# YiZhiXiaoGuLI/xerus

Measured on AMD Instinct MI355X. Metric: GFLOP/s on TT contraction + TT-round sweep time, order-10 rank-256, higher is better.
Workload: dtype f64; 1 GPU; TT order-10 n=20 rank-256: <x,y> + x.round(256) per step; order=10, mode_size=20, rank=256, parallelism=replicas x1

## Files before the change

include/xerus_amd.h:

```cpp
#ifndef XERUS_AMD_H
#define XERUS_AMD_H

#include <stddef.h>
#include <stdint.h>

#ifdef __cplusplus
extern "C" {
#endif

typedef struct xrs_handle_s* xrs_handle_t;

#define XRS_OK 0
#define XRS_EINVAL (-1)
#define XRS_ENOMEM (-2)
#define XRS_EHIP (-3)
#define XRS_ENUMERIC 1

int xrs_create(xrs_handle_t* handle, int device);
int xrs_destroy(xrs_handle_t handle);
int xrs_set_stream(xrs_handle_t handle, void* hip_stream);
void* xrs_get_stream(xrs_handle_t handle);
int xrs_synchronize(xrs_handle_t handle);
const char* xrs_last_error(void);
const char* xrs_version(void);
// ... 8 lines not shown

int xrs_nrm2(xrs_handle_t handle, double* result, const double* x, size_t n);
int xrs_dot(xrs_handle_t handle, double* result, const double* x, const double* y, size_t n);
int xrs_asum(xrs_handle_t handle, double* result, const double* x, size_t n);
int xrs_scal(xrs_handle_t handle, double* x, double alpha, size_t n);
int xrs_axpy(xrs_handle_t handle, double* y, double alpha, const double* x, size_t n);
int xrs_scale_rows(xrs_handle_t handle, double* X, const double* s, size_t m, size_t n);

int xrs_gemm(xrs_handle_t handle, double* C, size_t M, size_t N, double alpha,
             const double* A, size_t lda, int transA, size_t K,
             const double* B, size_t ldb, int transB);

int xrs_gemm_batched(xrs_handle_t handle, size_t count, double* const* C, size_t M, size_t N, double alpha,
                     const double* const* A, size_t lda, int transA, size_t K,
                     const double* const* B, size_t ldb, int transB);

int xrs_gemm_sym(xrs_handle_t handle, double* C, size_t N, double alpha,
                 const double* A, size_t lda, int transA, size_t K,
                 const double* B, size_t ldb, int transB);

int xrs_gemm_forms(xrs_handle_t handle, size_t count, double* const* C, size_t M, size_t N, double alpha,
                   const double* const* A, size_t lda, int transA, size_t K,
                   const double* const* B, size_t ldb, int transB, int sym, int tri);

int xrs_gemm_f32(xrs_handle_t handle, float* C, size_t M, size_t N, float alpha,
                 const float* A, size_t lda, int transA, size_t K,
                 const float* B, size_t ldb, int transB);

int xrs_permute(xrs_handle_t handle, double* out, const double* in, size_t ndim,
                const size_t* dims, const size_t* shuffle);

int xrs_qc(xrs_handle_t handle, double* Q, double* C, size_t* rank, const double* A, size_t m, size_t n);
int xrs_cq(xrs_handle_t handle, double* C, double* Q, size_t* rank, const double* A, size_t m, size_t n);
int xrs_qr(xrs_handle_t handle, double* Q, double* R, const double* A, size_t m, size_t n);
int xrs_rq(xrs_handle_t handle, double* R, double* Q, const double* A, size_t m, size_t n);
int xrs_svd(xrs_handle_t handle, double* U, double* S, double* Vt, const double* A, size_t m, size_t n);
int xrs_svd_batched(xrs_handle_t handle, double* U, double* S, double* Vt, int* status,
                    const double* A, size_t batch, size_t m, size_t n);
int xrs_svd_batched_fits(size_t m, size_t n);
int xrs_solve(xrs_handle_t handle, double* X, const double* A, size_t m, size_t n, const double* B, size_t p);
int xrs_solve_least_squares(xrs_handle_t handle, double* X, const double* A, size_t m, size_t n, const double* B, size_t p);
int xrs_svd_rows_vt(xrs_handle_t handle, double* S, double* Vt, int* sweeps, const double* A, size_t p, size_t q, int kernel);
int xrs_sym_tridiag(xrs_handle_t handle, double* d, double* e, const double* A, size_t n);
int xrs_sym_eig_top(xrs_handle_t handle, double* lam, double* Ut, int* status, const double* A, size_t n, size_t kk);


// ... 111 lines not shown
```

xerus_amd/capi.py:

```python
from __future__ import annotations

import ctypes as C
import os
from typing import Sequence

import numpy as np

_HERE = os.path.dirname(os.path.abspath(__file__))
LIB_PATH = os.environ.get("XRS_LIB_PATH") or os.path.join(_HERE, "libxerus_amd.so")

_SZ = C.c_size_t
_DP = C.c_void_p

SIGNATURES = {
    "xrs_create": (C.c_int, [C.POINTER(_DP), C.c_int]),
    "xrs_destroy": (C.c_int, [_DP]),
    "xrs_set_stream": (C.c_int, [_DP, _DP]),
    "xrs_get_stream": (_DP, [_DP]),
    "xrs_synchronize": (C.c_int, [_DP]),
    "xrs_last_error": (C.c_char_p, []),
    "xrs_version": (C.c_char_p, []),
    "xrs_malloc": (C.c_int, [_DP, C.POINTER(_DP), _SZ]),
    "xrs_free": (C.c_int, [_DP, _DP]),
    "xrs_pool_bytes": (_SZ, [_DP]),
    "xrs_upload": (C.c_int, [_DP, _DP, _DP, _SZ]),
    "xrs_download": (C.c_int, [_DP, _DP, _DP, _SZ]),
    "xrs_memset_zero": (C.c_int, [_DP, _DP, _SZ]),
    "xrs_copy": (C.c_int, [_DP, _DP, _DP, _SZ]),
    "xrs_nrm2": (C.c_int, [_DP, C.POINTER(C.c_double), _DP, _SZ]),
    "xrs_dot": (C.c_int, [_DP, C.POINTER(C.c_double), _DP, _DP, _SZ]),
    "xrs_asum": (C.c_int, [_DP, C.POINTER(C.c_double), _DP, _SZ]),
    "xrs_scal": (C.c_int, [_DP, _DP, C.c_double, _SZ]),
    "xrs_axpy": (C.c_int, [_DP, _DP, C.c_double, _DP, _SZ]),
    "xrs_scale_rows": (C.c_int, [_DP, _DP, _DP, _SZ, _SZ]),
    "xrs_gemm": (C.c_int, [_DP, _DP, _SZ, _SZ, C.c_double, _DP, _SZ, C.c_int, _SZ, _DP, _SZ, C.c_int]),
    "xrs_gemm_f32": (C.c_int, [_DP, _DP, _SZ, _SZ, C.c_float, _DP, _SZ, C.c_int, _SZ, _DP, _SZ, C.c_int]),
    "xrs_gemm_sym": (C.c_int,[_DP, _DP, _SZ, C.c_double, _DP, _SZ, C.c_int, _SZ, _DP, _SZ, C.c_int]),
    "xrs_gemm_batched": (C.c_int, [_DP, _SZ, C.POINTER(_DP), _SZ, _SZ, C.c_double, C.POINTER(_DP), _SZ, C.c_int, _SZ,
                                   C.POINTER(_DP), _SZ, C.c_int]),
    "xrs_gemm_forms": (C.c_int, [_DP, _SZ, C.POINTER(_DP), _SZ, _SZ, C.c_double, C.POINTER(_DP), _SZ, C.c_int, _SZ,
                                 C.POINTER(_DP), _SZ, C.c_int, C.c_int, C.c_int]),
    "xrs_permute": (C.c_int, [_DP, _DP, _DP, _SZ, C.POINTER(_SZ), C.POINTER(_SZ)]),
    "xrs_qc": (C.c_int, [_DP, _DP, _DP, C.POINTER(_SZ), _DP, _SZ, _SZ]),
    "xrs_cq": (C.c_int, [_DP, _DP, _DP, C.POINTER(_SZ), _DP, _SZ, _SZ]),
    "xrs_qr": (C.c_int, [_DP, _DP, _DP, _DP, _SZ, _SZ]),
    "xrs_rq": (C.c_int, [_DP, _DP, _DP, _DP, _SZ, _SZ]),
    "xrs_svd": (C.c_int, [_DP, _DP, _DP, _DP, _DP, _SZ, _SZ]),
    "xrs_svd_batched": (C.c_int, [_DP, _DP, _DP, _DP, C.POINTER(C.c_int), _DP, _SZ, _SZ, _SZ]),
    "xrs_svd_batched_fits": (C.c_int, [_SZ, _SZ]),
    "xrs_solve": (C.c_int, [_DP, _DP, _DP, _SZ, _SZ, _DP, _SZ]),
    "xrs_solve_least_squares": (C.c_int, [_DP, _DP, _DP, _SZ, _SZ, _DP, _SZ]),
    "xrs_svd_rows_vt": (C.c_int, [_DP, _DP, _DP, C.POINTER(C.c_int), _DP, _SZ, _SZ, C.c_int]),
    "xrs_sym_eig_top": (C.c_int, [_DP, _DP, _DP, C.POINTER(C.c_int), _DP, _SZ, _SZ]),
    "xrs_sym_tridiag": (C.c_int, [_DP, _DP, _DP, _DP, _SZ]),
    "xrs_tt_entrywise_product": (C.c_int, [_DP, _SZ, C.POINTER(_SZ), C.POINTER(_SZ), C.POINTER(_DP), C.POINTER(_SZ), C.POINTER(_DP),
                                           C.c_double, C.POINTER(_DP)]),
    "xrs_tt_entrywise_square": (C.c_int, [_DP, _SZ, C.POINTER(_SZ), C.POINTER(_SZ), C.POINTER(_DP), C.c_double, C.POINTER(_DP),
                                          C.POINTER(_SZ)]),
    "xrs_tt_rank_one_argmax": (C.c_int, [_DP, _SZ, C.POINTER(_SZ), C.POINTER(_DP), C.POINTER(_SZ)]),
    "xrs_tt_operator_apply": (C.c_int, [_DP, _SZ, C.POINTER(_SZ), C.POINTER(_SZ), C.POINTER(_SZ), C.POINTER(_SZ), C.POINTER(_DP),
                                        C.POINTER(_SZ), C.POINTER(_DP), C.c_int, C.POINTER(_DP)]),
    "xrs_tt_move_core": (C.c_int, [_DP, _SZ, C.POINTER(_SZ), C.POINTER(_SZ), C.POINTER(_DP), C.c_int, _SZ, _SZ, C.c_int]),
    "xrs_tt_round": (C.c_int, [_DP, _SZ, C.POINTER(_SZ), C.POINTER(_SZ), C.POINTER(_DP), C.c_int, _SZ,
                               C.POINTER(_SZ), C.c_double]),
# ... 159 lines not shown
    def gemm_f32(self, C_: "Float32Array", M, N, alpha, A: "Float32Array", lda, transA, K, B: "Float32Array", ldb, transB):
        _check("xrs_gemm_f32", self.lib.xrs_gemm_f32(self.h, _DP(C_.ptr), M, N, float(alpha), _DP(A.ptr), lda, int(transA),
                                                    K, _DP(B.ptr), ldb, int(transB)))

    def array_f32(self, a: np.ndarray) -> "Float32Array":
        return Float32Array.from_host(self, a)

    def gemm_sym(self, C_: "DeviceArray", N, alpha, A: "DeviceArray", lda, transA, K, B: "DeviceArray", ldb, transB):
        _check("xrs_gemm_sym", self.lib.xrs_gemm_sym(self.h, _DP(C_.ptr), N, alpha, _DP(A.ptr), lda, int(transA), K,
                                                    _DP(B.ptr), ldb, int(transB)))

    def gemm_batched(self, Cs, M, N, alpha, As, lda, transA, K, Bs, ldb, transB):
        cnt = len(Cs)
        tab = lambda xs: (_DP * max(1, cnt))(*[_DP(x.ptr) for x in xs])
        _check("xrs_gemm_batched", self.lib.xrs_gemm_batched(self.h, cnt, tab(Cs), M, N, alpha, tab(As), lda, int(transA),
                                                            K, tab(Bs), ldb, int(transB)))

    def gemm_forms(self, Cs, M, N, alpha, As, lda, transA, K, Bs, ldb, transB, sym: bool = False, tri: int = 0):
        cnt = len(Cs)
        tab = lambda xs: (_DP * max(1, cnt))(*[_DP(x.ptr) for x in xs])
        _check("xrs_gemm_forms", self.lib.xrs_gemm_forms(self.h, cnt, tab(Cs), M, N, alpha, tab(As), lda, int(transA), K,
                                                        tab(Bs), ldb, int(transB), int(sym), int(tri)))

    def tangent_to_tt(self, n, r, Us, Vs, add_base: bool):
        d = len(n)
        tab = lambda xs: (_DP * d)(*[_DP(x.ptr) for x in xs])
        out = (_DP * d)()
        _check("xrs_tt_tangent_to_tt", self.lib.xrs_tt_tangent_to_tt(self.h, d, _arr(n), _arr(r), tab(Us), tab(Vs),
                                                                    int(add_base), out))
        cores = []
        for k in range(d):
            shape = (2 * r[k] if k else 1, n[k], 2 * r[k + 1] if k + 1 < d else 1)
            c = DeviceArray(self, shape, ptr=out[k])
            c.owned = True
            cores.append(c)
        return cores

    def matmul(self, A: "DeviceArray", transA: bool, B: "DeviceArray", transB: bool, alpha: float = 1.0):
        am, ak = (A.shape[1], A.shape[0]) if transA else (A.shape[0], A.shape[1])
        bk, bn = (B.shape[1], B.shape[0]) if transB else (B.shape[0], B.shape[1])
        assert ak == bk, (A.shape, B.shape)
        out = self.empty((am, bn))
        self.gemm(out, am, bn, alpha, A, A.shape[1], transA, ak, B, B.shape[1], transB)
        return out

    def permute(self, out: "DeviceArray", inp: "DeviceArray", dims, shuffle):
# ... 495 lines not shown
```

xerus_amd/csrc/elementwise.hpp:

```cpp
#pragma once
#include <algorithm>

#include "runtime.hpp"

namespace xrs {

void reduce_to_device(xrs_handle_t h, int mode, const double* x, const double* y, size_t n, double* out_dev,
                      double* partial = nullptr);
double reduce_to_host(xrs_handle_t h, int mode, const double* x, const double* y, size_t n);
void scal(xrs_handle_t h, double* x, double alpha, size_t n);
void axpy(xrs_handle_t h, double* y, double alpha, const double* x, size_t n);
void ldexp_copy(xrs_handle_t h, double* dst, const double* src, int ex, size_t n);
constexpr int kAmaxMany = 64;
void amax_enqueue(xrs_handle_t h, const double* const* x, const size_t* n, int count, double* out_dev);
void norms_enqueue(xrs_handle_t h, const double* const* x, const size_t* n, int count, double* out_dev);
int range_exponent(double am);
int range_exponent(xrs_handle_t h, const double* A, size_t n);
void scale_rows(xrs_handle_t h, double* X, const double* s, size_t m, size_t n);
void scale_cols(xrs_handle_t h, double* X, const double* s, size_t m, size_t n);
void diag_sum(xrs_handle_t h, double* out, const double* X, size_t P, size_t m);
void offset_add(xrs_handle_t h, double* out, const size_t* out_dims, const double* in, const size_t* in_dims, size_t nd,
                const size_t* offsets, double alpha);
void strided_eval(xrs_handle_t h, double* out, const double* in, size_t nd, const size_t* out_dims, const size_t* in_strides,
                  size_t nt, const size_t* tr_dims, const size_t* tr_strides, size_t base);

constexpr int kTriA = 1, kTriB = 2;
void gemm(xrs_handle_t h, double* C, size_t M, size_t N, double alpha, const double* A, size_t lda, bool ta, size_t K,
          const double* B, size_t ldb, bool tb, int tri = 0);
constexpr int kGemmBatchMax = 32;
void gemm_batched(xrs_handle_t h, int count, double* const* C, size_t M, size_t N, double alpha, const double* const* A,
                  size_t lda, bool ta, size_t K, const double* const* B, size_t ldb, bool tb, bool sym = false,
                  int tri = 0);
void gemm_sym(xrs_handle_t h, double* C, size_t N, double alpha, const double* A, size_t lda, bool ta, size_t K,
              const double* B, size_t ldb, bool tb);

struct GemmSpec {
    const double* A;
    const double* B;
    double* C;
    size_t M, N, K, lda, ldb;
    bool ta, tb;
};
inline void gemm(xrs_handle_t h, const GemmSpec& g) {
    gemm(h, g.C, g.M, g.N, 1.0, g.A, g.lda, g.ta, g.K, g.B, g.ldb, g.tb);
}

void permute(xrs_handle_t h, double* out, const double* in, size_t ndim, const size_t* dims, const size_t* shuffle);

}
```

xerus_amd/csrc/gemm.hip:

```cpp
#include <algorithm>
#include <type_traits>
#include <utility>
#include <cstdio>
#include <cstdlib>

#include <hip/hip_ext.h>

#include "elementwise.hpp"
#include "runtime.hpp"

namespace xrs {

typedef double d4 __attribute__((ext_vector_type(4)));

struct GemmOne {
    const double* A;
    const double* B;
    double* C;
    __host__ __device__ const double* a(int) const { return A; }
    __host__ __device__ const double* b(int) const { return B; }
    __device__ double* c(int) const { return C; }
};
struct GemmMany {
    const double* A[kGemmBatchMax];
    const double* B[kGemmBatchMax];
    double* C[kGemmBatchMax];
    __host__ __device__ const double* a(int i) const { return A[i]; }
    __host__ __device__ const double* b(int i) const { return B[i]; }
    __device__ double* c(int i) const { return C[i]; }
};

template <int BM, int BN, int WGM, int WGN, int WGK>
constexpr int gemm_min_waves() { return (BM * BN >= 128 * 128) ? 2 : 4; }

#ifdef XRS_GEMM_TRACE
__device__ unsigned long long* g_gemm_trace = nullptr;
__device__ unsigned long long* g_gemm_steps = nullptr;
#define XRS_TRACE_BEGIN                                                   \
    const unsigned long long xrs_t0 = __builtin_amdgcn_s_memrealtime();  \
    const unsigned long long xrs_c0 = __builtin_amdgcn_s_memtime();
#define XRS_TRACE_STEP(t)                                                                                   \
    if (threadIdx.x == 0 && g_gemm_steps != nullptr && (t) < 15) {                                          \
        const size_t wg = blockIdx.x + size_t(gridDim.x) * (blockIdx.y + size_t(gridDim.y) * blockIdx.z);   \
        g_gemm_steps[16 * wg + (t)] = __builtin_amdgcn_s_memtime() - xrs_c0;                                \
    }
#define XRS_TRACE_END                                                                                     \
    if (threadIdx.x == 0 && g_gemm_trace != nullptr) {                                                    \
        const size_t wg = blockIdx.x + size_t(gridDim.x) * (blockIdx.y + size_t(gridDim.y) * blockIdx.z); \
        const unsigned long long t1 = __builtin_amdgcn_s_memrealtime();                                   \
        const unsigned hw = __builtin_amdgcn_s_getreg((31 << 11) | 4);                 \
        const unsigned xcc = __builtin_amdgcn_s_getreg((31 << 11) | 20);              \
        g_gemm_trace[3 * wg] = xrs_t0;                                                                   \
        g_gemm_trace[3 * wg + 1] = t1;                                                                   \
        g_gemm_trace[3 * wg + 2] = (static_cast<unsigned long long>(xcc) << 32) | hw;                    \
        if (g_gemm_steps != nullptr) g_gemm_steps[16 * wg + 15] = __builtin_amdgcn_s_memtime() - xrs_c0;  \
    }
#else
#define XRS_TRACE_BEGIN
#define XRS_TRACE_END
#define XRS_TRACE_STEP(t)
#endif

template <int BM, int BN, int GBK, int WGM, int WGN, int WGK, int PD, bool TA, bool TB, class PTR>
__device__ __forceinline__ void gemm_body(const PTR& ptrs, size_t lda, size_t ldb, int M, int N, int K, int kps,
                                          double alpha, double* __restrict__ slab, int tiles_m, int xcd_group,
                                          int* __restrict__ tickets, int sym);

template <int BM, int BN, int GBK, int WGM, int WGN, int WGK, int PD, bool TA, bool TB, class PTR>
__global__ void __launch_bounds__(WGM * WGN * WGK * 64, (gemm_min_waves<BM, BN, WGM, WGN, WGK>()))
k_gemm_f64(const PTR ptrs, size_t lda, size_t ldb, int M, int N, int K, int kps, double alpha,
           double* __restrict__ slab, int tiles_m, int xcd_group, int* __restrict__ tickets, int sym) {
    XRS_TRACE_BEGIN
    gemm_body<BM, BN, GBK, WGM, WGN, WGK, PD, TA, TB, PTR>(ptrs, lda, ldb, M, N, K, kps, alpha, slab, tiles_m,
                                                          xcd_group, tickets, sym);
    XRS_TRACE_END
}

template <int TM, int TN, int WGM, int WGN, int WGK, int NACC, class PTR>
__device__ __forceinline__ void gemm_finish(d4 (&acc2)[NACC][TM][TN], double* lds, const PTR& ptrs, int M, int N,
                                            double alpha, double* __restrict__ slab, int* __restrict__ tickets,
                                            int sym, int m0, int n0, int wm, int wn, int kg, int pos, int xb, int yb, int zb) {
    const int bz = yb;
    double* __restrict__ C = ptrs.c(bz);
    const int zslice = bz * int(gridDim.z) + zb;
    const int tslot = bz * int(gridDim.x) + xb;
    const int tid = threadIdx.x;
    const int lane = tid & 63;
    const bool mirror = sym != 0;
    d4 acc[TM][TN];
#pragma unroll
    for (int i = 0; i < TM; ++i)
#pragma unroll
        for (int j = 0; j < TN; ++j) {
            acc[i][j] = acc2[0][i][j];
            if constexpr (NACC > 1) acc[i][j] += acc2[1][i][j];
        }
    if constexpr (WGK > 1) {
        double* red = lds;
        if (kg > 0) {
#pragma unroll
            for (int i = 0; i < TM; ++i)
#pragma unroll
                for (int j = 0; j < TN; ++j)
#pragma unroll
                    for (int r = 0; r < 4; ++r)
                        red[((((kg - 1) * (WGM * WGN) + pos) * TM * TN + i * TN + j) * 4 + r) * 64 + lane] = acc[i][j][r];
        }
        __syncthreads();
// ... 23 lines not shown
#pragma unroll
                for (int r = 0; r < 4; ++r) {
                    const int row = m0 + wm + i * 16 + lg + 4 * r;
                    if (row < M && col < N) {
                        if (tickets != nullptr)
                            __hip_atomic_store(&out[size_t(row) * N + col], acc[i][j][r], __ATOMIC_RELAXED,
                                               __HIP_MEMORY_SCOPE_AGENT);
                        else if (!mirror || to_slab)
                            out[size_t(row) * N + col] = scale * acc[i][j][r];
                        else if (row >= col) {
                            out[size_t(row) * N + col] = scale * acc[i][j][r];
                            out[size_t(col) * N + row] = scale * acc[i][j][r];
                        }
                    }
                }
            }
    }
    if (tickets == nullptr) return;
    asm volatile("s_waitcnt vmcnt(0)" ::: "memory");
    __syncthreads();
    double* flag = lds;
    if (tid == 0) {
        const int t = __hip_atomic_fetch_add(&tickets[tslot], 1, __ATOMIC_RELAXED, __HIP_MEMORY_SCOPE_AGENT);
        const bool last = (t == int(gridDim.z) - 1);
        if (last) __hip_atomic_store(&tickets[tslot], 0, __ATOMIC_RELAXED, __HIP_MEMORY_SCOPE_AGENT);
        flag[0] = last ? 1.0 : 0.0;
    }
    __syncthreads();
    if (flag[0] == 0.0 || kg != 0) return;
#pragma unroll
    for (int i = 0; i < TM; ++i)
#pragma unroll
        for (int j = 0; j < TN; ++j) {
            const int col = n0 + wn + j * 16 + lc;
#pragma unroll
            for (int r = 0; r < 4; ++r) {
                const int row = m0 + wm + i * 16 + lg + 4 * r;
                if (row < M && col < N && (!mirror || row >= col)) {
                    const size_t o = size_t(row) * N + col;
                    double sum = 0.0;
                    for (int z = 0; z < int(gridDim.z); ++z)
                        sum += (z == zb) ? acc[i][j][r]
                                                      : __hip_atomic_load(&slab[(size_t(bz) * gridDim.z + z) * MN + o], __ATOMIC_RELAXED,
                                                                          __HIP_MEMORY_SCOPE_AGENT);
                    C[o] = alpha * sum;
                    if (mirror) C[size_t(col) * N + row] = alpha * sum;
                }
            }
        }
}


template <int BM, int BN, int GBK, int WGM, int WGN, int WGK, int PD, bool TA, bool TB, class PTR>
__device__ __forceinline__ void gemm_body(const PTR& ptrs, size_t lda, size_t ldb, int M, int N, int K, int kps,
                                          double alpha, double* __restrict__ slab, int tiles_m, int xcd_group,
                                          int* __restrict__ tickets, int sym) {
    const int bz = blockIdx.y;
    const double* __restrict__ A = ptrs.a(bz);
    const double* __restrict__ B = ptrs.b(bz);
    constexpr int NT = WGM * WGN * WGK * 64;
    constexpr int SA = BM;
    constexpr int SB = BN;
    static_assert(BM % 16 == 0 && BN % 16 == 0, "tile rows must be whole MFMA tiles");
    constexpr bool WIDE_SWZ_A = BM % 32 == 0, WIDE_SWZ_B = BN % 32 == 0;
    constexpr int WM = BM / WGM, WN = BN / WGN;
    constexpr int TM = WM / 16, TN = WN / 16;
    static_assert(TM >= 1 && TN >= 1, "wave tile smaller than one MFMA tile");
    constexpr int NACC = (TM * TN <= 2) ? 2 : 1;
    constexpr int A_PER = (BM * GBK + NT - 1) / NT;
    constexpr int B_PER = (BN * GBK + NT - 1) / NT;

    __shared__ double As[2][GBK * SA];
    __shared__ double Bs[2][GBK * SB];

    const int tid = threadIdx.x;
    const int lane = tid & 63;
    const int wave = tid >> 6;
    const int kg = wave / (WGM * WGN);
    const int pos = wave % (WGM * WGN);
    const int wm = (pos / WGN) * WM;
    const int wn = (pos % WGN) * WN;
    static_assert(GBK % (4 * WGK) == 0, "K-step must split evenly over the wave groups");
    static_assert(WGK == 1 || (WGK - 1) * BM * BN <= 2 * GBK * (SA + SB), "LDS reduction buffer too small");

    int tm, tn;
    {
        const int b = blockIdx.x, tiles_n = gridDim.x / tiles_m;
        if (xcd_group == 1) {
            const int xcd = b & 7, slot = b >> 3;
            tn = (slot / tiles_m) * 8 + xcd;
            tm = slot % tiles_m;
        } else if (xcd_group == 2) {
            const int xcd = b & 7, slot = b >> 3;
            tm = (slot / tiles_n) * 8 + xcd;
            tn = slot % tiles_n;
        } else {
            tm = b % tiles_m;
            tn = b / tiles_m;
        }
    }
    if (sym && tm < tn) return;
    const int m0 = tm * BM, n0 = tn * BN;
    const int kbeg = blockIdx.z * kps;
    const int kend = min(K, kbeg + kps);

    d4 acc2[NACC][TM][TN];
#pragma unroll
    for (int a = 0; a < NACC; ++a)
#pragma unroll
        for (int i = 0; i < TM; ++i)
#pragma unroll
            for (int j = 0; j < TN; ++j) acc2[a][i][j] = d4{0.0, 0.0, 0.0, 0.0};
    auto swza = [](int k) { return WIDE_SWZ_A ? (((k & 1) << 4) | (k & 15)) : (k & 15); };
    auto swzb = [](int k) { return WIDE_SWZ_B ? (((k & 1) << 4) | (k & 15)) : (k & 15); };

    double ra[PD][A_PER], rb[PD][B_PER];

    auto a_coord = [&](int e, int& m, int& k) {
        const int idx = tid + e * NT;
        if (TA) { m = idx % BM; k = idx / BM; } else { k = idx % GBK; m = idx / GBK; }
    };
    auto b_coord = [&](int e, int& n, int& k) {
        const int idx = tid + e * NT;
        if (TB) { k = idx % GBK; n = idx / GBK; } else { n = idx % BN; k = idx / BN; }
    };
    auto load_tile = [&](int k0, auto slot_c) {
// ... 68 lines not shown
                     load_tile(kbeg + (t + PD) * GBK, std::integral_constant<int, U>{});
                     __syncthreads();
                 }()),
                 ...);
            }(std::make_integer_sequence<int, PD>{});
        }
        for (; t0 < nsteps; t0 += PD) {
            [&]<int... U>(std::integer_sequence<int, U...>) {
                (([&] {
                     const int t = t0 + U;
                     if (t < nsteps) {
                         compute(U & 1);
                         if (t + 1 < nsteps)
                             store_tile((U + 1) & 1, kbeg + (t + 1) * GBK, std::integral_constant<int, (U + 1) % PD>{});
                         if (t + PD < nsteps) load_tile(kbeg + (t + PD) * GBK, std::integral_constant<int, U>{});
                     }
                     __syncthreads();
                 }()),
                 ...);
            }(std::make_integer_sequence<int, PD>{});
        }
    }

    gemm_finish<TM, TN, WGM, WGN, WGK, NACC>(acc2, &As[0][0], ptrs, M, N, alpha, slab, tickets, sym, m0, n0, wm, wn, kg, pos,
                                             int(blockIdx.x), int(blockIdx.y), int(blockIdx.z));
}

constexpr int kGldsBK = 32;

template <int R, bool KMAJ, int BK = kGldsBK>
struct GldsImg {
    static_assert(!KMAJ || R % 16 == 0, "k-major image rows must be whole MFMA tiles");
    static constexpr int KSWZ = (R % 32 == 0) ? 8 : 0;
    static constexpr int DOUBLES = R * BK;
    static constexpr int INSTR = DOUBLES * 8 / 1024;
    __device__ static int at(int r, int k) {
        if constexpr (!KMAJ) return r * BK + ((((k >> 1) ^ (r & 15))) << 1) + (k & 1);
        else return k * R + ((((r >> 1) ^ ((k & 1) * KSWZ))) << 1) + (r & 1);
    }
    template <int NF, int WGK>
    struct Frag {
        static_assert((WGK & (WGK - 1)) == 0, "wave groups must be a power of 2");
        int base[KMAJ ? NF : 1];
        int z = 0;
        __device__ Frag(int w0, int kg, int lane) {
            const int lr = lane & 15, lk = lane >> 4;
            if constexpr (!KMAJ) {
                base[0] = (w0 + lr) * BK + (lk & 1);
// ... 157 lines not shown
        double af[2][TM], bf[2][TN];
        auto frag = [&](int q, double(&a)[TM], double(&b)[TN]) {
#pragma unroll
            for (int i = 0; i < TM; ++i) a[i] = as[fa.off(q, i)];
#pragma unroll
            for (int j = 0; j < TN; ++j) b[j] = bs[fb.off(q, j)];
        };
        frag(0, af[0], bf[0]);
#ifndef XRS_GLDS_NOLOAD
        if (t + S - 1 < nsteps) issue(t + S - 1);
#endif
#pragma unroll
        for (int q = 0; q < NQ; ++q) {
            if (q + 1 < NQ) frag(q + 1, af[(q + 1) & 1], bf[(q + 1) & 1]);
            __builtin_amdgcn_sched_barrier(0);
#pragma unroll
            for (int i = 0; i < TM; ++i)
#pragma unroll
                for (int j = 0; j < TN; ++j)
                    acc2[q % NACC][i][j] = __builtin_amdgcn_mfma_f64_16x16x4f64(af[q & 1][i], bf[q & 1][j], acc2[q % NACC][i][j], 0, 0, 0);
        }
    }
    __syncthreads();
    gemm_finish<TM, TN, WGM, WGN, WGK, NACC>(acc2, lds, ptrs, M, N, alpha, slab, tickets, sym, m0, n0, wm, wn, kg, pos, xb, bz, zb);
}

template <int BM, int BN, int WGM, int WGN, int WGK, bool TA, bool TB, class PTR, int BK = kGldsBK, int ST = 0>
__global__ void __launch_bounds__(WGM * WGN * WGK * 64, (glds_min_waves<BM, BN, WGM, WGN, WGK>()))
k_gemm_glds(const PTR ptrs, size_t lda, size_t ldb, int M, int N, int K, int kps, double alpha,
            double* __restrict__ slab, int tiles_m, int xcd_group, int* __restrict__ tickets, int sym, int tri) {
    XRS_TRACE_BEGIN
    __shared__ double lds[glds_lds_doubles<BM, BN, BK, ST>()];
    glds_body<BM, BN, WGM, WGN, WGK, TA, TB, PTR, BK, ST>(lds, ptrs, lda, ldb, M, N, K, kps, alpha, slab, tiles_m, xcd_group,
                                                      tickets, sym, tri);
    XRS_TRACE_END
}

#ifndef XRS_REDUCE_CHUNK
#define XRS_REDUCE_CHUNK 16
#endif
constexpr int kReduceChunk = XRS_REDUCE_CHUNK;

__device__ __forceinline__ double slice_sum(const double* __restrict__ slab, size_t MN, int splits, size_t i) {
    double s = 0.0;
    for (int z0 = 0; z0 < splits; z0 += kReduceChunk) {
        double v[kReduceChunk];
#pragma unroll
// ... 315 lines not shown
}

void gemm_batched(xrs_handle_t h, int count, double* const* C, size_t Ms, size_t Ns, double alpha, const double* const* A,
                  size_t lda, bool ta, size_t Ks, const double* const* B, size_t ldb, bool tb, bool sym, int tri) {
    XRS_REQUIRE(!sym || Ms == Ns, "symmetric batch needs square results");
    if (Ms == 0 || Ns == 0 || count <= 0) return;
    XRS_REQUIRE(Ms < (1u << 30) && Ns < (1u << 30) && Ks < (1u << 30), "GEMM dimension too large");
    if (Ks == 0) {
        for (int i = 0; i < count; ++i) XRS_HIP(hipMemsetAsync(C[i], 0, Ms * Ns * 8, h->stream));
        return;
    }
    for (int b0 = 0; b0 < count; b0 += kGemmBatchMax) {
        const int c = std::min(kGemmBatchMax, count - b0);
        GemmMany P{};
        for (int i = 0; i < c; ++i) {
            P.A[i] = A[b0 + i];
            P.B[i] = B[b0 + i];
            P.C[i] = C[b0 + i];
        }
        gemm_impl(h, P, c, Ms, Ns, alpha, lda, ta, Ks, ldb, tb, sym, tri);
    }
}

}

#ifdef XRS_GEMM_TRACE
extern "C" int xrs_debug_gemm_trace(void* buf, void* steps) {
    unsigned long long* p = static_cast<unsigned long long*>(buf);
    unsigned long long* q = static_cast<unsigned long long*>(steps);
    return hipMemcpyToSymbol(HIP_SYMBOL(xrs::g_gemm_trace), &p, sizeof(p)) == hipSuccess &&
                   hipMemcpyToSymbol(HIP_SYMBOL(xrs::g_gemm_steps), &q, sizeof(q)) == hipSuccess
               ? 0 : 1;
}
#endif

extern "C" int xrs_gemm(xrs_handle_t h, double* C, size_t M, size_t N, double alpha, const double* A, size_t lda,
                        int transA, size_t K, const double* B, size_t ldb, int transB) {
    return xrs::guarded([&] {
        XRS_REQUIRE(h, "null handle");
        XRS_REQUIRE(M == 0 || N == 0 || C, "null C");
        XRS_REQUIRE(K == 0 || M == 0 || N == 0 || (A && B), "null A/B");
        XRS_REQUIRE(transA ? lda >= M || K == 0 : lda >= K || M == 0, "lda too small");
        XRS_REQUIRE(transB ? ldb >= K || N == 0 : ldb >= N || K == 0, "ldb too small");
        XRS_REQUIRE(C != A && C != B, "C must not alias A or B");
        xrs::fence_readers(h);
        xrs::gemm(h, C, M, N, alpha, A, lda, transA != 0, K, B, ldb, transB != 0);
// ... 60 lines not shown
```

xerus_amd/csrc/tt.hip:

```cpp
#include <algorithm>
#include <atomic>
#include <chrono>
#include <condition_variable>
#include <limits>
#include <mutex>
#include <thread>
#include <cstdio>
#include <cstdlib>
#include <cmath>
#include <string>
#include <vector>

#include "tt_common.hpp"

namespace xrs {

namespace ttd {


std::vector<size_t> maximal_ranks(const TT& t) {
    std::vector<size_t> rk(t.r + 1, t.r + t.d);
    size_t cur = 1;
    for (size_t i = 0; i + 1 < t.d; ++i) {
        cur *= t.n[i];
// ... 242 lines not shown
    for (int e = threadIdx.x + 256 * blockIdx.y; e < n * n; e += 256 * gridDim.y) {
        const double v = fabs(G[e] - ((e / n) == (e % n) ? 1.0 : 0.0));
        mx = (v > mx || v != v) ? v : mx;
    }
#pragma unroll
    for (int o = 32; o > 0; o >>= 1) {
        const double q = __shfl_xor(mx, o, 64);
        mx = (q > mx || q != q) ? q : mx;
    }
    if ((threadIdx.x & 63) == 0) red[threadIdx.x >> 6] = mx;
    __syncthreads();
    if (threadIdx.x == 0) {
        double m = red[0];
        for (int i = 1; i < 4; ++i) m = (red[i] > m || red[i] != red[i]) ? red[i] : m;
        args.out[blockIdx.x * gridDim.y + blockIdx.y] = m;
    }
}

void rl_sweep(TT& t, const size_t* max_ranks, double eps, double cX, size_t from);


void gemm_grouped(xrs_handle_t h, const std::vector<GemmJob>& jobs) {
    std::vector<bool> done(jobs.size(), false);
    for (size_t i = 0; i < jobs.size(); ++i) {
        if (done[i]) continue;
        const GemmJob& g = jobs[i];
        std::vector<const double*> A, B;
        std::vector<double*> C;
        for (size_t j = i; j < jobs.size(); ++j) {
            const GemmJob& o = jobs[j];
            if (done[j] || o.M != g.M || o.N != g.N || o.K != g.K || o.lda != g.lda || o.ldb != g.ldb || o.ta != g.ta ||
                o.tb != g.tb || o.sym != g.sym || o.alpha != g.alpha || o.tri != g.tri)
                continue;
            done[j] = true;
            A.push_back(o.A);
            B.push_back(o.B);
            C.push_back(o.C);
        }
        if (C.size() == 1 && g.sym) gemm_sym(h, C[0], g.N, g.alpha, A[0], g.lda, g.ta, g.K, B[0], g.ldb, g.tb);
        else if (C.size() == 1) gemm(h, C[0], g.M, g.N, g.alpha, A[0], g.lda, g.ta, g.K, B[0], g.ldb, g.tb, g.tri);
        else gemm_batched(h, int(C.size()), C.data(), g.M, g.N, g.alpha, A.data(), g.lda, g.ta, g.K, B.data(), g.ldb,
                          g.tb, g.sym, g.tri);
    }
}

struct ChainStatus {
    int* status = nullptr;
    int count = 0;
};

ChainStatus chain_pass(Sweep& sw, TT& t, bool certify, std::vector<double*>& C) {
    const size_t d = t.d;
    xrs_handle_t h = t.h;
    std::vector<double*> G, H;
    std::vector<DevBuf> gram_store, Lf(d);
    XRS_MARK("pass");
    gram_chains(t, G, H, gram_store, certify);
    open_dot_gate(h);
    XRS_MARK("chains");
    std::vector<DevBuf> Z(d), Cs;
// ... 543 lines not shown
           const size_t* max_ranks, double eps) {
    check_tt(d, n, r, cores);
    TT t{h, d, n, r, cores};
    xrs::round(t, canonicalized, core_pos, max_ranks, eps);
}
double dot(xrs_handle_t h, size_t d, const size_t* n, const size_t* rx, const double* const* X, const size_t* ry,
           const double* const* Y) {
    return xrs::dot(h, d, n, rx, X, ry, Y);
}
void soft_threshold(xrs_handle_t h, size_t d, const size_t* n, size_t* r, double** cores, bool canonicalized, size_t core_pos,
                    const double* taus) {
    check_tt(d, n, r, cores);
    TT t{h, d, n, r, cores};
    xrs::soft_threshold(t, canonicalized, core_pos, taus);
}
}

}

using namespace xrs;

extern "C" {

int xrs_tt_move_core(xrs_handle_t h, size_t d, const size_t* n, size_t* r, double** cores, int canonicalized,
                     size_t core_position, size_t position, int keep_rank) {
    return guarded([&] {
        XRS_REQUIRE(h, "null handle");
        check_tt(d, n, r, cores);
        XRS_REQUIRE(position < d, "Illegal core-position");
        XRS_REQUIRE(!canonicalized || core_position < d, "Illegal current core position");
        TT t{h, d, n, r, cores};
        move_core(t, canonicalized != 0, core_position, position, keep_rank != 0);
    });
}

int xrs_tt_round(xrs_handle_t h, size_t d, const size_t* n, size_t* r, double** cores, int canonicalized,
                 size_t core_position, const size_t* max_ranks, double eps) {
    return guarded([&] {
        XRS_REQUIRE(h, "null handle");
        check_tt(d, n, r, cores);
        XRS_REQUIRE(eps < 1.0 && eps >= 0.0, "_eps must be smaller than one.");
        for (size_t k = 0; k + 1 < d; ++k)
            XRS_REQUIRE(max_ranks[k] > 0, "Trying to round a TTTensor to rank 0 is not possible.");
        XRS_REQUIRE(!canonicalized || core_position < d, "Illegal current core position");
        TT t{h, d, n, r, cores};
        round(t, canonicalized != 0, core_position, max_ranks, eps);
// ... 107 lines not shown
```

Before: 36780 GFLOP/s.

## Batch small heterogeneous GEMMs into one ragged grouped kernel launch

Adds a ragged grouped GEMM kernel that packs several differently shaped small GEMMs (32x32 tiles, split-K with slab/ticket reduction) into a single launch via a kernel-argument table. gemm_grouped now routes singleton small groups of the same transpose class through this launch instead of issuing one GEMM launch each, aiming to cut launch overhead and poor occupancy for tiny contractions in TT sweeps. A public xrs_gemm_grouped entry point and Python binding are added. Risks are slower small-tile kernels for mid-size jobs and extra slab allocation per launch.

```diff
diff --git a/include/xerus_amd.h b/include/xerus_amd.h
--- a/include/xerus_amd.h
+++ b/include/xerus_amd.h
@@ -54,6 +54,10 @@
 int xrs_gemm_forms(xrs_handle_t handle, size_t count, double* const* C, size_t M, size_t N, double alpha,
                    const double* const* A, size_t lda, int transA, size_t K,
                    const double* const* B, size_t ldb, int transB, int sym, int tri);
+
+int xrs_gemm_grouped(xrs_handle_t handle, size_t count, double* const* C, const size_t* M, const size_t* N,
+                     const double* alpha, const double* const* A, const size_t* lda, int transA, const size_t* K,
+                     const double* const* B, const size_t* ldb, int transB, const int* sym);
 
 int xrs_gemm_f32(xrs_handle_t handle, float* C, size_t M, size_t N, float alpha,
                  const float* A, size_t lda, int transA, size_t K,
diff --git a/xerus_amd/capi.py b/xerus_amd/capi.py
--- a/xerus_amd/capi.py
+++ b/xerus_amd/capi.py
@@ -40,6 +40,9 @@
                                    C.POINTER(_DP), _SZ, C.c_int]),
     "xrs_gemm_forms": (C.c_int, [_DP, _SZ, C.POINTER(_DP), _SZ, _SZ, C.c_double, C.POINTER(_DP), _SZ, C.c_int, _SZ,
                                  C.POINTER(_DP), _SZ, C.c_int, C.c_int, C.c_int]),
+    "xrs_gemm_grouped": (C.c_int, [_DP, _SZ, C.POINTER(_DP), C.POINTER(_SZ), C.POINTER(_SZ), C.POINTER(C.c_double),
+                                   C.POINTER(_DP), C.POINTER(_SZ), C.c_int, C.POINTER(_SZ), C.POINTER(_DP), C.POINTER(_SZ),
+                                   C.c_int, C.POINTER(C.c_int)]),
     "xrs_permute": (C.c_int, [_DP, _DP, _DP, _SZ, C.POINTER(_SZ), C.POINTER(_SZ)]),
     "xrs_qc": (C.c_int, [_DP, _DP, _DP, C.POINTER(_SZ), _DP, _SZ, _SZ]),
     "xrs_cq": (C.c_int, [_DP, _DP, _DP, C.POINTER(_SZ), _DP, _SZ, _SZ]),
@@ -245,6 +248,15 @@
         _check("xrs_gemm_forms", self.lib.xrs_gemm_forms(self.h, cnt, tab(Cs), M, N, alpha, tab(As), lda, int(transA), K,
                                                         tab(Bs), ldb, int(transB), int(sym), int(tri)))
 
+    def gemm_grouped(self, jobs, transA, transB):
+        cnt = len(jobs)
+        tab = lambda k: (_DP * max(1, cnt))(*[_DP(j[k].ptr) for j in jobs])
+        szs = lambda k: (_SZ * max(1, cnt))(*[int(j[k]) for j in jobs])
+        alpha = (C.c_double * max(1, cnt))(*[float(j[3]) for j in jobs])
+        sym = (C.c_int * max(1, cnt))(*[int(bool(j[9])) for j in jobs])
+        _check("xrs_gemm_grouped", self.lib.xrs_gemm_grouped(self.h, cnt, tab(0), szs(1), szs(2), alpha, tab(4), szs(5),
+                                                            int(transA), szs(6), tab(7), szs(8), int(transB), sym))
+
     def tangent_to_tt(self, n, r, Us, Vs, add_base: bool):
         d = len(n)
         tab = lambda xs: (_DP * d)(*[_DP(x.ptr) for x in xs])
diff --git a/xerus_amd/csrc/elementwise.hpp b/xerus_amd/csrc/elementwise.hpp
--- a/xerus_amd/csrc/elementwise.hpp
+++ b/xerus_amd/csrc/elementwise.hpp
@@ -1,6 +1,7 @@
 #pragma once
 #include <algorithm>
 
+#include "gemm_ragged.hpp"
 #include "runtime.hpp"
 
 namespace xrs {
@@ -34,6 +35,17 @@
 void gemm_sym(xrs_handle_t h, double* C, size_t N, double alpha, const double* A, size_t lda, bool ta, size_t K,
               const double* B, size_t ldb, bool tb);
 
+struct RaggedJob {
+    const double* A;
+    const double* B;
+    double* C;
+    size_t M, N, K, lda, ldb;
+    double alpha;
+    bool sym;
+};
+const RaggedRule& gemm_ragged_rule();
+void gemm_ragged(xrs_handle_t h, const RaggedJob* jobs, int count, bool ta, bool tb);
+
 struct GemmSpec {
     const double* A;
     const double* B;
diff --git a/xerus_amd/csrc/gemm.hip b/xerus_amd/csrc/gemm.hip
--- a/xerus_amd/csrc/gemm.hip
+++ b/xerus_amd/csrc/gemm.hip
@@ -30,6 +30,20 @@
     __device__ double* c(int i) const { return C[i]; }
 };
 
+constexpr int kRaggedMax = 32;
+constexpr int kRaggedSumChunk = 8;
+struct GemmRagged {
+    const double* A[kRaggedMax];
+    const double* B[kRaggedMax];
+    double* C[kRaggedMax];
+    double alpha[kRaggedMax];
+    unsigned lda[kRaggedMax], ldb[kRaggedMax], slab[kRaggedMax];
+    int M[kRaggedMax], N[kRaggedMax], K[kRaggedMax];
+    int kps[kRaggedMax], splits[kRaggedMax], first[kRaggedMax], tick[kRaggedMax], sym[kRaggedMax];
+    int count;
+};
+static_assert(sizeof(GemmRagged) + 16 <= 4096, "kernel argument limit");
+
 template <int BM, int BN, int WGM, int WGN, int WGK>
 constexpr int gemm_min_waves() { return (BM * BN >= 128 * 128) ? 2 : 4; }
 
@@ -61,10 +75,10 @@
 #define XRS_TRACE_STEP(t)
 #endif
 
-template <int BM, int BN, int GBK, int WGM, int WGN, int WGK, int PD, bool TA, bool TB, class PTR>
+template <int BM, int BN, int GBK, int WGM, int WGN, int WGK, int PD, bool TA, bool TB, class PTR, bool RG = false>
 __device__ __forceinline__ void gemm_body(const PTR& ptrs, size_t lda, size_t ldb, int M, int N, int K, int kps,
                                           double alpha, double* __restrict__ slab, int tiles_m, int xcd_group,
-                                          int* __restrict__ tickets, int sym);
+                                          int* __restrict__ tickets, int sym, int xb, int yb, int zb, int nx, int nz);
 
 template <int BM, int BN, int GBK, int WGM, int WGN, int WGK, int PD, bool TA, bool TB, class PTR>
 __global__ void __launch_bounds__(WGM * WGN * WGK * 64, (gemm_min_waves<BM, BN, WGM, WGN, WGK>()))
@@ -72,18 +86,36 @@
            double* __restrict__ slab, int tiles_m, int xcd_group, int* __restrict__ tickets, int sym) {
     XRS_TRACE_BEGIN
     gemm_body<BM, BN, GBK, WGM, WGN, WGK, PD, TA, TB, PTR>(ptrs, lda, ldb, M, N, K, kps, alpha, slab, tiles_m,
-                                                          xcd_group, tickets, sym);
+                                                          xcd_group, tickets, sym, int(blockIdx.x), int(blockIdx.y),
+                                                          int(blockIdx.z), int(gridDim.x), int(gridDim.z));
     XRS_TRACE_END
 }
 
-template <int TM, int TN, int WGM, int WGN, int WGK, int NACC, class PTR>
+template <bool TA, bool TB>
+__global__ void __launch_bounds__(512, (gemm_min_waves<32, 32, 2, 2, 2>()))
+k_gemm_ragged(const GemmRagged tab, double* __restrict__ slab, int* __restrict__ tickets) {
+    const int b = int(blockIdx.x);
+    int e = 0;
+    while (e + 1 < tab.count && tab.first[e + 1] <= b) ++e;
+    const int M = tab.M[e], N = tab.N[e], nz = tab.splits[e];
+    const int tiles_m = (M + 31) / 32, tiles = tiles_m * ((N + 31) / 32);
+    const int local = b - tab.first[e];
+    const GemmOne one{tab.A[e], tab.B[e], tab.C[e]};
+    gemm_body<32, 32, 16, 2, 2, 2, 2, TA, TB, GemmOne, true>(one, tab.lda[e], tab.ldb[e], M, N, tab.K[e], tab.kps[e], tab.alpha[e],
+                                                             nz > 1 ? slab + tab.slab[e] : nullptr, tiles_m, 0,
+                                                             nz > 1 ? tickets + tab.tick[e] : nullptr, tab.sym[e],
+                                                             local % tiles, 0, local / tiles, tiles, nz);
+}
+
+template <int TM, int TN, int WGM, int WGN, int WGK, int NACC, class PTR, bool RG = false>
 __device__ __forceinline__ void gemm_finish(d4 (&acc2)[NACC][TM][TN], double* lds, const PTR& ptrs, int M, int N,
                                             double alpha, double* __restrict__ slab, int* __restrict__ tickets,
-                                            int sym, int m0, int n0, int wm, int wn, int kg, int pos, int xb, int yb, int zb) {
+                                            int sym, int m0, int n0, int wm, int wn, int kg, int pos, int xb, int yb, int zb,
+                                            int nx, int nz) {
     const int bz = yb;
     double* __restrict__ C = ptrs.c(bz);
-    const int zslice = bz * int(gridDim.z) + zb;
-    const int tslot = bz * int(gridDim.x) + xb;
+    const int zslice = bz * nz + zb;
+    const int tslot = bz * nx + xb;
     const int tid = threadIdx.x;
     const int lane = tid & 63;
     const bool mirror = sym != 0;
@@ -153,12 +185,46 @@
     double* flag = lds;
     if (tid == 0) {
         const int t = __hip_atomic_fetch_add(&tickets[tslot], 1, __ATOMIC_RELAXED, __HIP_MEMORY_SCOPE_AGENT);
-        const bool last = (t == int(gridDim.z) - 1);
+        const bool last = (t == nz - 1);
         if (last) __hip_atomic_store(&tickets[tslot], 0, __ATOMIC_RELAXED, __HIP_MEMORY_SCOPE_AGENT);
         flag[0] = last ? 1.0 : 0.0;
     }
     __syncthreads();
     if (flag[0] == 0.0 || kg != 0) return;
+    if constexpr (RG) {
+        static_assert(TM == 1 && TN == 1, "ragged combine: one MFMA tile per wave");
+        const int col = n0 + wn + lc;
+        size_t o[4];
+        bool ok[4];
+        double sum[4] = {0.0, 0.0, 0.0, 0.0};
+#pragma unroll
+        for (int r = 0; r < 4; ++r) {
+            const int row = m0 + wm + lg + 4 * r;
+            ok[r] = row < M && col < N && (!mirror || row >= col);
+            o[r] = ok[r] ? size_t(row) * N + col : 0;
+        }
+        for (int z0 = 0; z0 < nz; z0 += kRaggedSumChunk) {
+            double v[kRaggedSumChunk][4];
+#pragma unroll
+            for (int u = 0; u < kRaggedSumChunk; ++u)
+#pragma unroll
+                for (int r = 0; r < 4; ++r)
+                    v[u][r] = __hip_atomic_load(&slab[size_t(min(z0 + u, nz - 1)) * MN + o[r]], __ATOMIC_RELAXED,
+                                                __HIP_MEMORY_SCOPE_AGENT);
+#pragma unroll
+            for (int u = 0; u < kRaggedSumChunk; ++u)
+#pragma unroll
+                for (int r = 0; r < 4; ++r)
+                    if (z0 + u < nz) sum[r] += (z0 + u == zb) ? acc[0][0][r] : v[u][r];
+        }
+#pragma unroll
+        for (int r = 0; r < 4; ++r)
+            if (ok[r]) {
+                C[o[r]] = alpha * sum[r];
+                if (mirror) C[size_t(col) * N + (m0 + wm + lg + 4 * r)] = alpha * sum[r];
+            }
+        return;
+    }
 #pragma unroll
     for (int i = 0; i < TM; ++i)
 #pragma unroll
@@ -170,9 +236,9 @@
                 if (row < M && col < N && (!mirror || row >= col)) {
                     const size_t o = size_t(row) * N + col;
                     double sum = 0.0;
-                    for (int z = 0; z < int(gridDim.z); ++z)
+                    for (int z = 0; z < nz; ++z)
                         sum += (z == zb) ? acc[i][j][r]
-                                                      : __hip_atomic_load(&slab[(size_t(bz) * gridDim.z + z) * MN + o], __ATOMIC_RELAXED,
+                                                      : __hip_atomic_load(&slab[(size_t(bz) * unsigned(nz) + z) * MN + o], __ATOMIC_RELAXED,
                                                                           __HIP_MEMORY_SCOPE_AGENT);
                     C[o] = alpha * sum;
                     if (mirror) C[size_t(col) * N + row] = alpha * sum;
@@ -182,11 +248,11 @@
 }
 
 
-template <int BM, int BN, int GBK, int WGM, int WGN, int WGK, int PD, bool TA, bool TB, class PTR>
+template <int BM, int BN, int GBK, int WGM, int WGN, int WGK, int PD, bool TA, bool TB, class PTR, bool RG>
 __device__ __forceinline__ void gemm_body(const PTR& ptrs, size_t lda, size_t ldb, int M, int N, int K, int kps,
                                           double alpha, double* __restrict__ slab, int tiles_m, int xcd_group,
-                                          int* __restrict__ tickets, int sym) {
-    const int bz = blockIdx.y;
+                                          int* __restrict__ tickets, int sym, int xb, int yb, int zb, int nx, int nz) {
+    const int bz = yb;
     const double* __restrict__ A = ptrs.a(bz);
     const double* __restrict__ B = ptrs.b(bz);
     constexpr int NT = WGM * WGN * WGK * 64;
@@ -216,7 +282,7 @@
 
     int tm, tn;
     {
-        const int b = blockIdx.x, tiles_n = gridDim.x / tiles_m;
+        const int b = xb, tiles_n = unsigned(nx) / tiles_m;
         if (xcd_group == 1) {
             const int xcd = b & 7, slot = b >> 3;
             tn = (slot / tiles_m) * 8 + xcd;
@@ -232,7 +298,7 @@
     }
     if (sym && tm < tn) return;
     const int m0 = tm * BM, n0 = tn * BN;
-    const int kbeg = blockIdx.z * kps;
+    const int kbeg = zb * kps;
     const int kend = min(K, kbeg + kps);
 
     d4 acc2[NACC][TM][TN];
@@ -347,8 +413,8 @@
         }
     }
 
-    gemm_finish<TM, TN, WGM, WGN, WGK, NACC>(acc2, &As[0][0], ptrs, M, N, alpha, slab, tickets, sym, m0, n0, wm, wn, kg, pos,
-                                             int(blockIdx.x), int(blockIdx.y), int(blockIdx.z));
+    gemm_finish<TM, TN, WGM, WGN, WGK, NACC, PTR, RG>(acc2, &As[0][0], ptrs, M, N, alpha, slab, tickets, sym, m0, n0, wm, wn,
+                                                      kg, pos, xb, yb, zb, nx, nz);
 }
 
 constexpr int kGldsBK = 32;
@@ -552,7 +618,8 @@
         }
     }
     __syncthreads();
-    gemm_finish<TM, TN, WGM, WGN, WGK, NACC>(acc2, lds, ptrs, M, N, alpha, slab, tickets, sym, m0, n0, wm, wn, kg, pos, xb, bz, zb);
+    gemm_finish<TM, TN, WGM, WGN, WGK, NACC>(acc2, lds, ptrs, M, N, alpha, slab, tickets, sym, m0, n0, wm, wn, kg, pos, xb, bz, zb,
+                                             int(gridDim.x), int(gridDim.z));
 }
 
 template <int BM, int BN, int WGM, int WGN, int WGK, bool TA, bool TB, class PTR, int BK = kGldsBK, int ST = 0>
@@ -914,6 +981,56 @@
     }
 }
 
+const RaggedRule& gemm_ragged_rule() {
+    static const RaggedRule rule = [] {
+        RaggedRule r;
+        if (const char* e = std::getenv("XRS_GEMM_RAGGED")) std::sscanf(e, "%d,%d,%d", &r.cut, &r.slice, &r.max_slices);
+        return r;
+    }();
+    return rule;
+}
+
+void gemm_ragged(xrs_handle_t h, const RaggedJob* jobs, int count, bool ta, bool tb) {
+    const RaggedRule& rule = gemm_ragged_rule();
+    std::vector<RaggedShape> shapes(static_cast<size_t>(std::max(count, 0)));
+    for (int i = 0; i < count; ++i) {
+        shapes[i] = {jobs[i].M, jobs[i].N, jobs[i].K, jobs[i].lda, jobs[i].ldb};
+        XRS_REQUIRE(ragged_small(shapes[i], rule), "job outside the ragged launch's range");
+        XRS_REQUIRE(!jobs[i].sym || jobs[i].M == jobs[i].N, "symmetric result needs M == N");
+    }
+    for (int b0 = 0; b0 < count;) {
+        RaggedEntry plan[kRaggedMax];
+        const RaggedChunk ch = ragged_plan(shapes.data(), count, b0, rule, kRaggedMax, xrs_handle_s::kTicketCap, plan);
+        GemmRagged T{};
+        double flops = 0.0, bytes = 0.0;
+        for (int i = 0; i < ch.count; ++i) {
+            const RaggedJob& j = jobs[b0 + i];
+            T.A[i] = j.A, T.B[i] = j.B, T.C[i] = j.C;
+            T.alpha[i] = j.alpha;
+            T.lda[i] = unsigned(j.lda), T.ldb[i] = unsigned(j.ldb), T.slab[i] = plan[i].slab;
+            T.M[i] = int(j.M), T.N[i] = int(j.N), T.K[i] = int(j.K);
+            T.kps[i] = plan[i].kps, T.splits[i] = plan[i].splits, T.first[i] = plan[i].first, T.tick[i] = plan[i].tick;
+            T.sym[i] = j.sym ? 1 : 0;
+            flops += 2.0 * double(j.M) * double(j.N) * double(j.K);
+            bytes += 8.0 * (double(j.M) * j.K + double(j.K) * j.N + double(j.M) * j.N * plan[i].splits);
+        }
+        T.count = ch.count;
+        DevBuf slab;
+        if (ch.slab_doubles > 0) slab = DevBuf(h, ch.slab_doubles * sizeof(double));
+        KernelTimer timer(h, XRS_KFAM_GEMM, flops, bytes, true);
+#define XRS_RAGGED_LAUNCH(TA_, TB_)                                                                                  \
+    hipExtLaunchKernelGGL((k_gemm_ragged<TA_, TB_>), dim3(unsigned(ch.workgroups)), dim3(512), 0, h->stream, timer.start(), \
+                          timer.stop(), 0, T, slab.d(), h->tickets)
+        if (!ta && !tb) XRS_RAGGED_LAUNCH(false, false);
+        else if (!ta && tb) XRS_RAGGED_LAUNCH(false, true);
+        else if (ta && !tb) XRS_RAGGED_LAUNCH(true, false);
+        else XRS_RAGGED_LAUNCH(true, true);
+#undef XRS_RAGGED_LAUNCH
+        check_launch("k_gemm_ragged");
+        b0 += ch.count;
+    }
+}
+
 }
 
 #ifdef XRS_GEMM_TRACE
diff --git a/xerus_amd/csrc/gemm_ragged.hpp b/xerus_amd/csrc/gemm_ragged.hpp
--- /dev/null
+++ b/xerus_amd/csrc/gemm_ragged.hpp
@@ -0,0 +1,84 @@
+#pragma once
+#include <algorithm>
+#include <cstddef>
+
+namespace xrs {
+
+constexpr int kRaggedTile = 32;
+constexpr int kRaggedStep = 16;
+
+struct RaggedRule {
+    int cut = 512, slice = 256, max_slices = 32;
+};
+
+struct RaggedShape {
+    size_t M, N, K, lda, ldb;
+};
+
+inline size_t ragged_tiles(size_t M, size_t N) {
+    return ((M + kRaggedTile - 1) / kRaggedTile) * ((N + kRaggedTile - 1) / kRaggedTile);
+}
+
+inline bool ragged_small(const RaggedShape& s, const RaggedRule& r) {
+    if (s.M == 0 || s.N == 0 || s.K == 0) return false;
+    if (s.M >= (1u << 30) || s.N >= (1u << 30) || s.K >= (1u << 30)) return false;
+    if (s.lda > 0xffffffffull || s.ldb > 0xffffffffull) return false;
+    return ragged_tiles(s.M, s.N) < size_t(r.cut);
+}
+
+inline void ragged_slices(size_t K, const RaggedRule& r, int& splits, int& kps) {
+    const size_t slice = size_t(std::max(r.slice, kRaggedStep));
+    size_t s = std::min<size_t>((K + slice - 1) / slice, size_t(std::max(r.max_slices, 1)));
+    s = std::max<size_t>(s, 1);
+    size_t d = (K + s - 1) / s;
+    d = (d + kRaggedStep - 1) / kRaggedStep * kRaggedStep;
+    kps = int(d);
+    splits = int((K + d - 1) / d);
+}
+
+struct RaggedEntry {
+    int splits, kps, first, tick;
+    unsigned slab;
+};
+struct RaggedChunk {
+    int count = 0;
+    int workgroups = 0;
+    int tickets = 0;
+    size_t slab_doubles = 0;
+};
+
+inline RaggedChunk ragged_plan(const RaggedShape* shapes, int count, int begin, const RaggedRule& rule, int max_entries,
+                               int ticket_cap, RaggedEntry* out) {
+    RaggedChunk c;
+    for (int i = begin; i < count && c.count < max_entries; ++i) {
+        const RaggedShape& s = shapes[i];
+        const size_t tiles = ragged_tiles(s.M, s.N);
+        RaggedEntry e{1, 0, c.workgroups, 0, 0};
+        ragged_slices(s.K, rule, e.splits, e.kps);
+        if (e.splits > 1 && tiles > size_t(ticket_cap)) {
+            e.splits = 1;
+            e.kps = int((s.K + kRaggedStep - 1) / kRaggedStep * kRaggedStep);
+        }
+        if (e.splits > 1) {
+            const size_t need = size_t(e.splits) * s.M * s.N;
+            const bool full = size_t(c.tickets) + tiles > size_t(ticket_cap) || c.slab_doubles + need > 0x7fffffffull;
+            if (full && c.count > 0) break;
+            if (full) {
+                e.splits = 1;
+                e.kps = int((s.K + kRaggedStep - 1) / kRaggedStep * kRaggedStep);
+            } else {
+                e.tick = c.tickets;
+                e.slab = unsigned(c.slab_doubles);
+                c.tickets += int(tiles);
+                c.slab_doubles += need;
+            }
+        }
+        const size_t wgs = tiles * size_t(e.splits);
+        if (size_t(c.workgroups) + wgs > 0x3fffffffull && c.count > 0) break;
+        out[c.count++] = e;
+        c.workgroups += int(wgs);
+    }
+    return c;
+}
+
+}
diff --git a/xerus_amd/csrc/tt.hip b/xerus_amd/csrc/tt.hip
--- a/xerus_amd/csrc/tt.hip
+++ b/xerus_amd/csrc/tt.hip
@@ -288,20 +288,47 @@
 
 void gemm_grouped(xrs_handle_t h, const std::vector<GemmJob>& jobs) {
     std::vector<bool> done(jobs.size(), false);
+    std::vector<std::vector<size_t>> groups;
     for (size_t i = 0; i < jobs.size(); ++i) {
         if (done[i]) continue;
         const GemmJob& g = jobs[i];
-        std::vector<const double*> A, B;
-        std::vector<double*> C;
+        groups.emplace_back();
         for (size_t j = i; j < jobs.size(); ++j) {
             const GemmJob& o = jobs[j];
             if (done[j] || o.M != g.M || o.N != g.N || o.K != g.K || o.lda != g.lda || o.ldb != g.ldb || o.ta != g.ta ||
                 o.tb != g.tb || o.sym != g.sym || o.alpha != g.alpha || o.tri != g.tri)
                 continue;
             done[j] = true;
-            A.push_back(o.A);
-            B.push_back(o.B);
-            C.push_back(o.C);
+            groups.back().push_back(j);
+        }
+    }
+    std::vector<bool> ragged(groups.size(), false);
+    const RaggedRule& rule = gemm_ragged_rule();
+    for (int cls = 0; cls < 4 && rule.cut > 0; ++cls) {
+        const bool ta = (cls & 2) != 0, tb = (cls & 1) != 0;
+        std::vector<RaggedJob> small;
+        std::vector<size_t> from;
+        for (size_t q = 0; q < groups.size(); ++q) {
+            const GemmJob& g = jobs[groups[q][0]];
+            if (groups[q].size() != 1 || g.ta != ta || g.tb != tb || (g.sym && g.M != g.N) ||
+                !ragged_small({g.M, g.N, g.K, g.lda, g.ldb}, rule))
+                continue;
+            small.push_back({g.A, g.B, g.C, g.M, g.N, g.K, g.lda, g.ldb, g.alpha, g.sym});
+            from.push_back(q);
+        }
+        if (small.size() < 2) continue;
+        gemm_ragged(h, small.data(), int(small.size()), ta, tb);
+        for (size_t q : from) ragged[q] = true;
+    }
+    for (size_t q = 0; q < groups.size(); ++q) {
+        if (ragged[q]) continue;
+        const GemmJob& g = jobs[groups[q][0]];
+        std::vector<const double*> A, B;
+        std::vector<double*> C;
+        for (size_t j : groups[q]) {
+            A.push_back(jobs[j].A);
+            B.push_back(jobs[j].B);
+            C.push_back(jobs[j].C);
         }
         if (C.size() == 1 && g.sym) gemm_sym(h, C[0], g.N, g.alpha, A[0], g.lda, g.ta, g.K, B[0], g.ldb, g.tb);
         else if (C.size() == 1) gemm(h, C[0], g.M, g.N, g.alpha, A[0], g.lda, g.ta, g.K, B[0], g.ldb, g.tb, g.tri);
@@ -891,6 +918,29 @@
 
 extern "C" {
 
+int xrs_gemm_grouped(xrs_handle_t h, size_t count, double* const* C, const size_t* M, const size_t* N, const double* alpha,
+                     const double* const* A, const size_t* lda, int transA, const size_t* K, const double* const* B,
+                     const size_t* ldb, int transB, const int* sym) {
+    return guarded([&] {
+        XRS_REQUIRE(h, "null handle");
+        XRS_REQUIRE(count == 0 || (A && B && C && M && N && K && lda && ldb && alpha && sym), "null table");
+        XRS_REQUIRE(count < (1u << 20), "group too large");
+        std::vector<ttd::GemmJob> jobs;
+        for (size_t i = 0; i < count; ++i) {
+            XRS_REQUIRE(M[i] < (1u << 30) && N[i] < (1u << 30) && K[i] < (1u << 30), "GEMM dimension too large");
+            XRS_REQUIRE(M[i] == 0 || N[i] == 0 || C[i], "null C");
+            XRS_REQUIRE(K[i] == 0 || M[i] == 0 || N[i] == 0 || (A[i] && B[i]), "null A/B");
+            XRS_REQUIRE(transA ? lda[i] >= M[i] || K[i] == 0 : lda[i] >= K[i] || M[i] == 0, "lda too small");
+            XRS_REQUIRE(transB ? ldb[i] >= K[i] || N[i] == 0 : ldb[i] >= N[i] || K[i] == 0, "ldb too small");
+            XRS_REQUIRE(!sym[i] || M[i] == N[i], "symmetric result needs M == N");
+            XRS_REQUIRE(C[i] != A[i] && C[i] != B[i], "C must not alias A or B");
+            jobs.push_back({M[i], N[i], K[i], lda[i], ldb[i], transA != 0, transB != 0, A[i], B[i], C[i], sym[i] != 0, alpha[i]});
+        }
+        fence_readers(h);
+        ttd::gemm_grouped(h, jobs);
+    });
+}
+
 int xrs_tt_move_core(xrs_handle_t h, size_t d, const size_t* n, size_t* r, double** cores, int canonicalized,
                      size_t core_position, size_t position, int keep_rank) {
     return guarded([&] {
```

New measurement: 37400 GFLOP/s (median of 6 runs). About the same (+1.7%).
